# PeterCalifano/gtsam_PeterCdev

Measured on AMD Instinct MI355X. Metric: lm_iterations_per_sec, higher is better.
Workload: dtype f64; 1 GPU; bal1723; ordering=schur_nd, replicas=1, parallelism=replicas1

## Files before the change

### gtsam_petercdev_amd/csrc/handle.h

```cpp
#pragma once
#include <hip/hip_runtime.h>

#include <algorithm>
#include <new>
#include <stdexcept>
#include <string>
#include <utility>
#include <vector>

#include "gsx_internal.h"
#include "kernels.h"

#define HIPCHK(ctx, expr)                                                                  \
  do {                                                                                     \
    hipError_t e__ = (expr);                                                               \
    if (e__ != hipSuccess) {                                                               \
      (ctx)->err = std::string(#expr) + ": " + hipGetErrorString(e__);                     \
      return GSX_E_NO_DEVICE;                                                              \
    }                                                                                      \
  } while (0)

namespace gsx {

template <class Tp>
// ... 40 lines not shown
};

enum Phase { PH_LINEARIZE, PH_ASSEMBLE_H, PH_FACTORIZE, PH_BACKSOLVE, PH_LINERR, PH_RETRACT, PH_ERROR,
             PH_FACTOR_SMALL, PH_FACTOR_BIG, PH_FACTOR_LEAF, PH_K_SYRK, PH_K_TRSM, PH_K_POTRF0, PH_K_GATHER,
             PH_K_BACKSOLVE, PH_MARGINALS, PH_M_PREP, PH_M_KT, PH_M_SF, PH_M_FF, PH_M_EMIT, PH_M_LEAF, PH_COUNT };

struct Timer {
  std::vector<std::pair<hipEvent_t, hipEvent_t>> pending, pool;
  double ms = 0;
  int64_t count = 0;
};

}

namespace gsx {

struct Context {
  std::string err;
  int device = 0;
  bool has_device = false;
  hipStream_t stream = nullptr;
  HostProblem P;
  Symbolic S;
  bool has_symbolic = false;
  double relax = GSX_AMALGAMATION_AUTO;
  int relax_max_f = 128;
  std::vector<int> order;

  DevBuf<int> d_var_type, d_var_dim, d_var_state_off, d_var_tan_off, d_f_type, d_f_rows, d_f_key_ptr, d_f_vars,
      d_f_noise_kind, d_f_cols;
  DevBuf<i64> d_f_meas_off, d_f_noise_off, d_f_jac_off;
  DevBuf<double> d_meas, d_noise;
  DevBuf<FactorRec> d_frec;
  DevBuf<int> d_type_list[kNumTypeLists];
  int type_count[kNumTypeLists] = {};
  DevProblem DP{};
  int n_smart = 0;
  DevBuf<int> d_smart_slot, d_smart_status, d_smart_counters;
  DevBuf<double> d_smart_cams, d_smart_cache, d_smart_point;
  SmartDev SD{};
  void smart_begin(bool linearize) {
    if (n_smart) hipMemsetAsync(d_smart_counters.p + (linearize ? 0 : 1), 0, (linearize ? 2 : 1) * sizeof(int), stream);
  }
  DevBuf<i64> d_fr_off, d_cmap_ptr, d_gidx_ptr, d_h_off, d_hmap_ptr, d_term_ptr;
  DevBuf<TermRec> d_terms;
  DevBuf<VarRec> d_var_recs;
  DevBuf<ChildRec> d_child_recs;
  DevBuf<FrontRec> d_front_recs;
  DevBuf<i64> d_cond_last, d_cond_prev;
  DevBuf<int> d_cond_front;
  DevBuf<VarRec> d_fvar_recs;
  DevBuf<LeafRec> d_leaf_recs;
  int leaf_base = 0;
  int lin_err_slice = 0;
  DevBuf<int> d_fr_N, d_fr_F, d_fr_nfv, d_fr_fvar_ptr, d_fvars, d_fr_parent, d_fr_lean, d_fr_child_ptr, d_children, d_cmap,
      d_gidx, d_h_rows, d_hmap, d_h_loc, d_sched, d_hvars;
  DevBuf<BigDesc> d_big;
  DevSymbolic DS{};
  std::vector<std::vector<SmallLaunch>> small_launch;
  std::vector<std::vector<SmallLaunch>> leaf_launch;
  std::vector<int> leaf_max_F;
  std::vector<std::vector<SmallLaunch>> rest_launch;
  DevBuf<int> d_usched, d_rest_ids, d_tree_start, d_tree_up, d_tree_npend, d_tree_pending, d_tree_cursor;
  DevBuf<int> d_bst_roots, d_bst_child_ptr, d_bst_children, d_bst_counters;
  DevBuf<unsigned long long> d_bst_ready;
  int bst_roots = 0, bst_total = 0;
  unsigned bst_epoch = 0;
  struct TreeTier {
    int start0, nstart, max_n, threads;
    size_t med_lds;
  };
  std::vector<TreeTier> tree_tiers;
  DevBuf<i64> d_gt_dst;
  DevBuf<GatherSeg> d_gsegs;
  DevBuf<GatherSrc> d_gsrcs;
  DevBuf<int> d_gt_ld, d_gt_dims, d_gm_task, d_gm_slot, d_gm_nslots;
  DevBuf<double> d_gscratch;
  GatherArgs GA{};
  std::vector<BigLevel> big_level;
  struct ConLevel {
    int first = 0, count = 0, max_n = 0;
  };
  std::vector<ConLevel> con_level;
  std::vector<int> con_desc_of_front;
  DevBuf<ConDesc> d_con_descs;
  DevBuf<int> d_con_own_col_ptr, d_con_own_cols, d_con_own_m, d_con_child, d_con_fwd_map, d_con_iwork;
  DevBuf<i64> d_con_own_jac;
  DevBuf<double> d_con_work;
  ConTables CT{};
  int con_hd_n = 0;
  DevBuf<int> d_con_hd_tan, d_con_hd_ptr;
  DevBuf<i64> d_con_hd_jidx;
  DevBuf<double> d_con_hd_w;
  bool constrained() const { return !S.con_fronts.empty(); }
  std::vector<BigDesc> big_descs;
  int big_max_n = 0, big_max_nfv = 0;
  struct HGroup {
    int begin, count, threads, lds;
    bool global;
  };
  std::vector<HGroup> hgroups;
  DevBuf<int2> d_star_bundles;
  int n_star_bundles = 0;
  bool fused_star_env = true;
  bool fused_star = false;
  struct LeafSplit {
// ... 251 lines not shown
```

### gtsam_petercdev_amd/csrc/kernels.h

```cpp
#pragma once
#include <hip/hip_runtime.h>

#include <cstdint>
#include <vector>

#include "../../include/gsx.h"

namespace gsx {

typedef long long i64;

struct FactorRec {
  i64 jac_off;
  int s0, s1;
  int meas_off, noise_off;
  int type_kind;
  int rows_dim;
};
struct DevProblem {
  int n_vars, n_factors;
  const int *var_type, *var_dim, *var_state_off, *var_tan_off;
  const int *f_type, *f_rows, *f_key_ptr, *f_vars, *f_noise_kind, *f_cols;
  const i64 *f_meas_off, *f_noise_off, *f_jac_off;
  const double *meas, *noise;
  const FactorRec* frec;
  const int* f_active;
  int n_active;
};

struct TermRec {
  i64 jac;
  int m, colA, colB, dB, dst, pad;
};

struct VarRec {
  i64 h_off, hmap_off;
  int dA, rows, loc, toff;
};
struct LeafRec {
  i64 off, h_off, hmap_off, gidx_ptr;
  int n, F, nfv, lean;
  int dA, rows, loc, toff;
  int fvar_ptr, front, pad0, pad1;
};
constexpr int kStarMaxD = 3;
struct StarLeafRec {
  i64 off, h_off, t0;
  i64 jac0, prow_off;
  int n, nf, d, toff;
  int colA, colB, colR, dB;
  int front, jstride, rrow, pad0;
};
struct ChildRec {
  i64 src0, cmap_off;
  int nc, s1, pad0, pad1;
};
struct FrontRec {
  i64 off;
  int n, F, nfv, fvar_ptr, child_ptr, nchild;
};

struct DevSymbolic {
  int n_fronts;
  const i64* fr_off;
  const int *fr_N, *fr_F, *fr_nfv, *fr_fvar_ptr, *fvars, *fr_parent, *fr_child_ptr, *children;
  const int* fr_lean;
  const i64 *cmap_ptr, *gidx_ptr;
  const int *cmap, *gidx;
  const i64 *h_off, *hmap_ptr;
  const int *h_rows, *hmap, *h_loc;
  const i64* term_ptr;
  const TermRec* terms;
  const VarRec* var_recs;
  const ChildRec* child_recs;
  const FrontRec* front_recs;
  const VarRec* fvar_recs;
  unsigned char* wf_dirty;
  const unsigned char *wf_replaced, *wf_changed;
};
#ifdef __HIPCC__
__device__ __forceinline__ bool wildfire_skip(const DevSymbolic& S, int f, bool writer) {
  if (S.wf_dirty == nullptr) return false;
  const int p = S.fr_parent[f];
  bool dirty = (p < 0) || S.wf_dirty[p];
  if (dirty && !S.wf_replaced[f]) {
    dirty = false;
    for (int q = S.fr_fvar_ptr[f] + S.fr_nfv[f]; q < S.fr_fvar_ptr[f + 1]; ++q)
      if (S.wf_changed[S.fvars[q]]) {
        dirty = true;
        break;
      }
  }
  if (writer) S.wf_dirty[f] = dirty ? 1 : 0;
  return !dirty;
}
#endif

// ... 124 lines not shown
void launch_front_leaf(const DevProblem& P, const DevSymbolic& S, const LeafRec* recs, int count, int max_panel, int threads,
                       const double* H, const double* damp, const double* scalars, double* arena, DevStatus* status,
                       hipStream_t st);
void launch_front_star_leaf(const DevSymbolic& S, const StarLeafRec* recs, int count, const int* prow, const double* jac,
                            const double* damp, const double* scalars, double* H, double* arena, DevStatus* status,
                            hipStream_t st);
struct GatherSrc {
  i64 off;
  int d2;
  int ldF;
};
struct GatherSeg {
  i64 dst;
  i64 src;
  int n, ld, dims;
  int slot;
};
struct GatherArgs {
  const GatherSeg* segs;
  const GatherSrc* srcs;
  const i64* gt_dst;
  const int *gt_ld, *gt_dims, *gm_task, *gm_slot, *gm_nslots;
  double* scratch;
};
void launch_big_gather(const GatherArgs& G, int seg0, int nseg, int m0, int nm, double* arena, hipStream_t st);
void launch_backsolve(const DevSymbolic& S, const int* ids, int count, int threads, int max_n, const double* arena,
                      double* delta, DevStatus* status, hipStream_t st);
size_t backsolve_big_lds(int max_n, int max_F, int max_sep_rows);
void launch_backsolve_big(const DevSymbolic& S, const int* ids, int count, int max_n, int max_F, const double* arena,
                          double* delta, DevStatus* status, hipStream_t st);
bool backsolve_small_fits(int max_n, int max_F);
void launch_backsolve_small(const DevSymbolic& S, const int* ids, int count, int max_F, const double* arena, double* delta,
                            DevStatus* status, hipStream_t st);
struct BacksolveTreeArgs {
  const int* roots;
  int n_roots, n_tickets;
  const int *child_ptr, *children;
  unsigned long long* ready;
  int *head, *tail;
  unsigned epoch;
};
void launch_backsolve_tree(const DevSymbolic& S, const BacksolveTreeArgs& Q, const double* arena, double* delta,
                           DevStatus* status, hipStream_t st);
struct WildfireArgs {
  const unsigned char *replaced, *dirty;
  unsigned char* changed;
  const double* old_delta;
  DevStatus* status;
  double threshold;
};
void launch_mark_fronts(const int* ids, int count, unsigned char* flags, hipStream_t st);
void launch_wildfire_post(const DevSymbolic& S, const int* ids, int count, bool wave_per_clique, const WildfireArgs& W,
                          double* delta, hipStream_t st);
void launch_backsolve_leaf(const DevSymbolic& S, const LeafRec* recs, int count, int max_F, const double* arena,
                           double* delta, DevStatus* status, hipStream_t st);
void launch_gradient(const DevProblem& P, const DevSymbolic& S, const double* H, double* g, hipStream_t st);
void launch_ax_sqnorm(const DevProblem& P, const double* jac, const double* x, double* partials, int cap, double* scalars,
                      int slot, hipStream_t st);
void launch_vec_dot(const double* a, const double* b, int64_t n, double* partials, int cap, double* scalars, int slot,
                    hipStream_t st);
void launch_vec_axpby(double* out, double alpha, const double* a, double beta, const double* b, int64_t n, hipStream_t st);
void launch_marginal_path(const DevSymbolic& S, const int* path, int npath, int loc, int dA, int max_n, const double* arena,
                          double* out, double* Y, int64_t n_tan, hipStream_t st);
void launch_joint_cross(const double* Ya, const double* Yb, int64_t n_tan, int dA, int dB, double* out, hipStream_t st);
struct MargItem {
  int front, ti, tj, pad;
};
struct MargArgs {
  const i64 *slot, *work;
  double* cov;
  const double* arena;
  const i64* out_off;
  const int* var_dim;
  double* out;
};
void launch_marg_prep(const DevSymbolic& S, const MargArgs& M, const MargItem* items, int count, hipStream_t st);
void launch_marg_kt(const DevSymbolic& S, const MargArgs& M, const MargItem* items, int count, hipStream_t st);
void launch_marg_sf(const DevSymbolic& S, const MargArgs& M, const MargItem* items, int count, hipStream_t st);
void launch_marg_ff(const DevSymbolic& S, const MargArgs& M, const MargItem* items, int count, hipStream_t st);
void launch_marg_emit(const DevSymbolic& S, const MargArgs& M, const int2* vars, int count, hipStream_t st);
void launch_marg_leaf(const DevSymbolic& S, const MargArgs& M, const int* ids, int count, hipStream_t st);
void launch_set_scalar(double* scalars, int slot, double v, hipStream_t st);
struct ConDesc {
  i64 off;
  i64 work, fwd;
  i64 iwork;
  int N, F, K, n_fwd;
  int own_begin, own_end;
  int child_begin, child_end;
  int front;
  int fwd_map;
};
struct ConTables {
  const ConDesc* descs;
  const int *own_col_ptr, *own_cols, *own_m;
  const i64* own_jac;
  const int* child_list;
  const int* fwd_map;
  double* work;
  int* iwork;
};
void launch_constraint_fronts(const DevSymbolic& S, const ConTables& T, int first, int count, int max_n, const double* jac,
                              double* arena, DevStatus* status, hipStream_t st);
void launch_constraint_hdiag(int n, const int* tan, const int* ptr, const i64* jidx, const double* w, const double* jac,
                             double* hdiag, hipStream_t st);
constexpr int kTreeCursors = 8;
void launch_begin_factorization(double* scalars, double lambda, DevStatus* status, int* tree_cursors, hipStream_t st);
void launch_dense_partial(double* a, int n, int nf, DevStatus* status, hipStream_t st);
// ... 25 lines not shown
```

### gtsam_petercdev_amd/csrc/kernels.hip

```cpp
#include <hip/hip_runtime.h>

#include <climits>
#include <cstdio>
#include <cstdlib>

#include "device_geometry.h"
#include "gsx_internal.h"
#include "kernels.h"

namespace gsx {
using namespace gsxd;

#define T kTile

__device__ __forceinline__ double wave_sum(double v) {
#pragma unroll
  for (int o = 32; o > 0; o >>= 1) v += __shfl_down(v, o, 64);
  return v;
}
typedef double v4d __attribute__((ext_vector_type(4)));
__device__ __forceinline__ i64 readlane_i64(i64 v, int src_lane) {
  int lo = (int)(v & 0xFFFFFFFFll), hi = (int)(v >> 32);
  lo = __builtin_amdgcn_readlane(lo, src_lane);
  hi = __builtin_amdgcn_readlane(hi, src_lane);
// ... 3161 lines not shown
        acc0 += col0[r] * x;
        acc1 += col1[r] * x;
      }
#pragma unroll
      for (int o = 32; o > 0; o >>= 1) {
        acc0 += __shfl_down(acc0, o, 64);
        acc1 += __shfl_down(acc1, o, 64);
      }
      if (lane == 0) {
        y[c] = col0[n - 1] - acc0;
        if (two) y[c + 1] = col1[n - 1] - acc1;
      }
    }
#pragma unroll
    for (int q = 0; q < kTR; ++q) {
      const int e = tid + q * nt;
      if (e < w * w) {
        int r, c;
        divmod_small(e, w, rw, c, r);
        tile[r][c] = treg[q];
      }
    }
    if (tid < w) dv[tid] = dreg;
    __syncthreads();
    if (wave == 0) {
      double yr;
      if (has_inv) {
        yr = 0;
        if (lane < w) {
          yr = y[lane] * dv[lane];
          for (int r = lane + 1; r < w; ++r) yr += tile[lane][r] * y[r];
        }
      } else {
        yr = (lane < w) ? y[lane] : 0.0;
        for (int c = w - 1; c >= 0; --c) {
          const double xc = __shfl(yr, c, 64) / tile[c][c];
          if (lane == c) yr = xc;
          else if (lane < c) yr -= tile[c][lane] * xc;
        }
      }
      if (lane < w) xs[c0 + lane] = yr;
    }
    lds_barrier();
  }
  int bad = 0;
  for (int r = tid; r < F; r += nt) {
    const double x = xs[r];
    delta[gi[r]] = x;
    if (!isfinite(x)) bad = 1;
  }
  if (bad) atomicAdd(&status->n_nonfinite, 1);
}
template <int FM>
__global__ void __launch_bounds__(256) backsolve_leaf_kernel(DevSymbolic S, const LeafRec* recs, int count,
                                                             const double* arena, double* delta, DevStatus* status) {
  const int lane = threadIdx.x & 63;
  const int k = __builtin_amdgcn_readfirstlane(blockIdx.x * 4 + (threadIdx.x >> 6));
  if (k >= count) return;
  const LeafRec rec = recs[k];
  if (wildfire_skip(S, rec.front, lane == 0)) return;
  const int n = rec.n, F = rec.F;
  const double* A = arena + rec.off;
  const int* gi = S.gidx + rec.gidx_ptr;
  constexpr int U = 2;
  int g[U];
  double a[U][FM];
#pragma unroll
  for (int u = 0; u < U; ++u) {
    const int r = F + lane + 64 * u;
    const bool ok = r < n - 1;
    g[u] = ok ? gi[r] : -1;
#pragma unroll
    for (int c = 0; c < FM; ++c) a[u][c] = (ok && c < F) ? A[r + (i64)c * n] : 0.0;
  }
  const int gf = lane < F ? gi[lane] : -1;
  const int tr = lane % max(F, 1), tc = lane / max(F, 1);
  const double tri = (FM <= 8 && tc < F) ? A[tr + (i64)tc * n] : 0.0;
  const double dl = lane < F ? A[(n - 1) + (i64)lane * n] : 0.0;
  double yc[FM];
#pragma unroll
  for (int c = 0; c < FM; ++c) yc[c] = 0.0;
#pragma unroll
  for (int u = 0; u < U; ++u) {
    const double x = g[u] >= 0 ? delta[g[u]] : 0.0;
#pragma unroll
    for (int c = 0; c < FM; ++c) yc[c] = fma(a[u][c], x, yc[c]);
  }
  for (int r = F + lane + 64 * U; r < n - 1; r += 64) {
    const double x = delta[gi[r]];
#pragma unroll
    for (int c = 0; c < FM; ++c)
      if (c < F) yc[c] += A[r + (i64)c * n] * x;
  }
#pragma unroll
  for (int c = 0; c < FM; ++c) {
#pragma unroll
    for (int o = 32; o > 0; o >>= 1) yc[c] += __shfl_xor(yc[c], o, 64);
    yc[c] = tile_readlane(dl, c) - yc[c];
  }
  double xv[FM];
#pragma unroll
  for (int c = FM - 1; c >= 0; --c) {
    xv[c] = 0.0;
    if (c < F) {
      double acc = yc[c];
#pragma unroll
      for (int r = c + 1; r < FM; ++r)
        if (r < F) acc -= (FM <= 8 ? tile_readlane(tri, r + c * F) : A[r + (i64)c * n]) * xv[r];
      xv[c] = acc / (FM <= 8 ? tile_readlane(tri, c + c * F) : A[c + (i64)c * n]);
    }
  }
  double mine = 0.0;
#pragma unroll
  for (int c = 0; c < FM; ++c) mine = (lane == c) ? xv[c] : mine;
  if (lane < F) {
    delta[gf] = mine;
    if (!isfinite(mine)) atomicAdd(&status->n_nonfinite, 1);
  }
}

void launch_backsolve_leaf(const DevSymbolic& S, const LeafRec* recs, int count, int max_F, const double* arena,
                           double* delta, DevStatus* status, hipStream_t st) {
  if (!count) return;
  const int grid = (count + 3) / 4;
  if (max_F <= 4) backsolve_leaf_kernel<4><<<grid, 256, 0, st>>>(S, recs, count, arena, delta, status);
  else if (max_F <= 8) backsolve_leaf_kernel<8><<<grid, 256, 0, st>>>(S, recs, count, arena, delta, status);
  else backsolve_leaf_kernel<kLeafMaxF><<<grid, 256, 0, st>>>(S, recs, count, arena, delta, status);
}

template <bool WAVE>
__global__ void __launch_bounds__(256) wildfire_post_kernel(DevSymbolic S, const int* ids, int count, WildfireArgs W,
                                                            double* delta) {
  __shared__ int solved;
  if (threadIdx.x == 0) solved = 0;
  __syncthreads();
  const int lane = WAVE ? (threadIdx.x & 63) : 0, step = WAVE ? 64 : 1;
  const int k = WAVE ? blockIdx.x * 4 + (threadIdx.x >> 6) : blockIdx.x * 256 + threadIdx.x;
  if (k < count && W.dirty[ids[k]]) {
    const int f = ids[k];
    const int F = S.fr_F[f], nfv = S.fr_nfv[f];
    const int* gi = S.gidx + S.gidx_ptr[f];
    if (lane == 0) atomicAdd(&solved, nfv);
    bool keep = W.replaced[f] != 0;
    if (!keep) {
      double m = 0.0;
      for (int r = lane; r < F; r += step) {
        const int g = gi[r];
        m = fmax(m, fabs(W.old_delta[g] - delta[g]));
      }
      keep = WAVE ? (bool)__any(m >= W.threshold) : (m >= W.threshold);
    }
    if (keep) {
      for (int q = lane; q < nfv; q += step) W.changed[S.fvars[S.fr_fvar_ptr[f] + q]] = 1;
    } else {
      for (int r = lane; r < F; r += step) {
        const int g = gi[r];
        delta[g] = W.old_delta[g];
      }
    }
  }
  __syncthreads();
  if (threadIdx.x == 0 && solved) atomicAdd(&W.status->n_backsub, solved);
}
void launch_wildfire_post(const DevSymbolic& S, const int* ids, int count, bool wave_per_clique, const WildfireArgs& W,
                          double* delta, hipStream_t st) {
  if (count <= 0) return;
  if (wave_per_clique) wildfire_post_kernel<true><<<(count + 3) / 4, 256, 0, st>>>(S, ids, count, W, delta);
  else wildfire_post_kernel<false><<<(count + 255) / 256, 256, 0, st>>>(S, ids, count, W, delta);
}
__global__ void __launch_bounds__(256) mark_fronts_kernel(const int* ids, int count, unsigned char* flags) {
  const int k = blockIdx.x * blockDim.x + threadIdx.x;
  if (k < count) flags[ids[k]] = 1;
}
void launch_mark_fronts(const int* ids, int count, unsigned char* flags, hipStream_t st) {
  if (count > 0) mark_fronts_kernel<<<(count + 255) / 256, 256, 0, st>>>(ids, count, flags);
}

void launch_backsolve(const DevSymbolic& S, const int* ids, int count, int threads, int max_n, const double* arena,
                      double* delta, DevStatus* status, hipStream_t st) {
  static bool attr = false;
// ... 74 lines not shown
```

### gtsam_petercdev_amd/csrc/solver.hip

```cpp
#include <hip/hip_runtime.h>

#include <algorithm>
#include <cstdlib>
#include <chrono>
#include <climits>
#include <cmath>
#include <cstdio>
#include <cstring>
#include <limits>
#include <array>
#include <map>
#include <string>
#include <vector>

#include "handle.h"

using namespace gsx;

using namespace gsx;

namespace gsx {

void launch_lds_group(const DevProblem& P, const DevSymbolic& S, const int* ids, const SmallLaunch& g, const double* H,
                      const double* damp, const double* scalars, double* arena, DevStatus* status, hipStream_t st) {
// ... 221 lines not shown
    if (c->profiling > 0) timer_begin(c, PH_FACTOR_SMALL);
    const TreeArgs ta{c->d_tree_start.p + tt.start0, tt.nstart, c->d_tree_cursor.p + t, c->d_tree_pending.p,
                      c->d_tree_up.p, c->d_tree_npend.p};
    if (tt.med_lds)
      launch_front_tree_med(c->DP, c->DS, ta, tt.med_lds, c->d_H.p, c->d_damp.p, c->d_scalars.p, c->d_arena.p,
                            c->d_status.p, c->stream);
    else
      launch_front_tree(c->DP, c->DS, ta, tt.max_n, tt.threads, c->d_H.p, c->d_damp.p, c->d_scalars.p, c->d_arena.p,
                        c->d_status.p, c->stream);
    debug_sync(c, tt.med_lds ? "front_tree_med" : "front_tree", tt.nstart, (int)tt.med_lds);
    if (c->profiling > 0) timer_end(c, PH_FACTOR_SMALL);
  }
  for (int l = 0; l < S.n_ulevels; ++l) {
    for (const SmallLaunch& sl : c->rest_launch[l]) {
      if (c->profiling > 0) timer_begin(c, PH_FACTOR_SMALL);
      launch_lds_group(c->DP, c->DS, c->d_rest_ids.p + sl.begin, sl, c->d_H.p, c->d_damp.p, c->d_scalars.p, c->d_arena.p,
                       c->d_status.p, c->stream);
      debug_sync(c, sl.medium ? "front_medium (level)" : "front_small (level)", sl.count, sl.medium ? sl.max_panel : sl.max_n);
      if (c->profiling > 0) timer_end(c, PH_FACTOR_SMALL);
    }
    if (have_side && l == S.side_level0 + 1 && c->bulk_pending) {
      hipStreamWaitEvent(c->stream, c->bulk_done, 0);
      c->bulk_pending = false;
    }
    const BigLevel& B = c->big_level[l];
    const bool prof = c->profiling > 0;
    if (prof && B.count) timer_begin(c, PH_FACTOR_BIG);
    if (S.gseg_lvl_ptr[l + 1] > S.gseg_lvl_ptr[l]) {
      if (prof) timer_begin(c, PH_K_GATHER);
      launch_big_gather(c->GA, S.gseg_lvl_ptr[l], S.gseg_lvl_ptr[l + 1] - S.gseg_lvl_ptr[l], S.gm_lvl_ptr[l],
                        S.gm_lvl_ptr[l + 1] - S.gm_lvl_ptr[l], c->d_arena.p, c->stream);
      if (prof) timer_end(c, PH_K_GATHER);
    }
    if (l == 0 && have_side && !use_bulk && S.gseg_lvl_ptr[sg + 1] > S.gseg_lvl_ptr[sg]) {
      if (prof) timer_begin(c, PH_K_GATHER);
      launch_big_gather(c->GA, S.gseg_lvl_ptr[sg], S.gseg_lvl_ptr[sg + 1] - S.gseg_lvl_ptr[sg], S.gm_lvl_ptr[sg],
                        S.gm_lvl_ptr[sg + 1] - S.gm_lvl_ptr[sg], c->d_arena.p, c->stream);
      if (prof) timer_end(c, PH_K_GATHER);
    }
    if (B.count) {
      if (l == S.cap_ulevel0) shard_allreduce(c, c->d_arena.p + S.cap_begin, S.cap_end - S.cap_begin);
      if (c->con_level[l].count)
        launch_constraint_fronts(c->DS, c->CT, c->con_level[l].first, c->con_level[l].count, c->con_level[l].max_n,
                                 c->d_jac.p, c->d_arena.p, c->d_status.p, c->stream);
      dev_big_factor(c, c->d_big.p + B.begin, B.count, B.plan, c->stream, prof);
      if (prof) timer_end(c, PH_FACTOR_BIG);
    }
  }
  launch_cond_check((int)S.cond_last.size(), c->d_cond_last.p, c->d_cond_prev.p, c->d_cond_front.p, c->d_arena.p,
                    c->d_status.p, c->stream);
  timer_end(c, PH_FACTORIZE);
}

static void dev_backsolve_levels(gsx_context* c, const WildfireArgs* wf) {
  const Symbolic& S = c->S;
  timer_begin(c, PH_BACKSOLVE);
  c->delta_overwritten();
  for (int l = S.n_levels - 1; l >= 0; --l) {
    const int se = S.lvl_small_end[l];
    const struct {
      int count;
    } B{S.lvl_ptr[l + 1] - se};
    const int le = S.lvl_leaf_end[l], n_rest = S.lvl_ptr[l + 1] - le;
    int big_maxn = 0, big_maxF = 0, big_maxS = 0;
    for (int k = se; k < S.lvl_ptr[l + 1]; ++k) {
      big_maxn = std::max(big_maxn, S.N[S.sched[k]]);
      big_maxF = std::max(big_maxF, S.F[S.sched[k]]);
      big_maxS = std::max(big_maxS, S.N[S.sched[k]] - S.F[S.sched[k]]);
    }
    const bool big_own = B.count > 0 && backsolve_big_lds(big_maxn, big_maxF, big_maxS) > 0;
    if (big_own) {
      if (c->profiling > 0) timer_begin(c, PH_K_BACKSOLVE);
      launch_backsolve_big(c->DS, c->d_sched.p + se, S.lvl_ptr[l + 1] - se, big_maxn, big_maxF, c->d_arena.p, c->d_delta.p,
                           c->d_status.p, c->stream);
      if (c->profiling > 0) timer_end(c, PH_K_BACKSOLVE);
    }
    const int* small_ids = c->d_sched.p + le;
    const int n_small = se - le;
    int small_maxn = 0, small_maxF = 0;
    for (int k = le; k < se; ++k) {
      small_maxn = std::max(small_maxn, S.N[S.sched[k]]);
      small_maxF = std::max(small_maxF, S.F[S.sched[k]]);
    }
    const bool small_own = n_small > 0 && backsolve_small_fits(small_maxn, small_maxF);
    if (small_own) {
      if (c->profiling > 0) timer_begin(c, PH_K_BACKSOLVE);
      launch_backsolve_small(c->DS, small_ids, n_small, small_maxF, c->d_arena.p, c->d_delta.p, c->d_status.p,
                             c->stream);
      if (c->profiling > 0) timer_end(c, PH_K_BACKSOLVE);
    }
    const bool big_left = B.count > 0 && !big_own, small_left = n_small > 0 && !small_own;
    if (big_left && small_left && n_rest <= 512 && n_rest > B.count) {
      int maxn = 0;
      for (int k = le; k < S.lvl_ptr[l + 1]; ++k) maxn = std::max(maxn, S.N[S.sched[k]]);
      if (c->profiling > 0) timer_begin(c, PH_K_BACKSOLVE);
      launch_backsolve(c->DS, c->d_sched.p + le, n_rest, 1024, maxn, c->d_arena.p, c->d_delta.p, c->d_status.p, c->stream);
      if (c->profiling > 0) timer_end(c, PH_K_BACKSOLVE);
    } else {
      if (big_left) {
        int maxn = 0;
        for (int k = se; k < S.lvl_ptr[l + 1]; ++k) maxn = std::max(maxn, S.N[S.sched[k]]);
        if (c->profiling > 0) timer_begin(c, PH_K_BACKSOLVE);
        launch_backsolve(c->DS, c->d_sched.p + se, S.lvl_ptr[l + 1] - se, 1024, maxn, c->d_arena.p, c->d_delta.p,
                         c->d_status.p, c->stream);
        if (c->profiling > 0) timer_end(c, PH_K_BACKSOLVE);
      }
      if (small_left) {
        if (c->profiling > 0) timer_begin(c, PH_K_BACKSOLVE);
        launch_backsolve(c->DS, small_ids, n_small, small_maxn <= 48 ? 64 : 256, small_maxn, c->d_arena.p,
                         c->d_delta.p, c->d_status.p, c->stream);
        if (c->profiling > 0) timer_end(c, PH_K_BACKSOLVE);
      }
    }
    if (S.lvl_leaf_end[l] > S.lvl_ptr[l])
      launch_backsolve_leaf(c->DS, c->d_leaf_recs.p + (S.lvl_ptr[l] - c->leaf_base), S.lvl_leaf_end[l] - S.lvl_ptr[l],
                            c->leaf_max_F[l], c->d_arena.p, c->d_delta.p, c->d_status.p, c->stream);
    if (wf) {
      launch_wildfire_post(c->DS, c->d_sched.p + S.lvl_ptr[l], le - S.lvl_ptr[l], false, *wf, c->d_delta.p, c->stream);
      launch_wildfire_post(c->DS, c->d_sched.p + le, n_rest, true, *wf, c->d_delta.p, c->stream);
    }
  }
  timer_end(c, PH_BACKSOLVE);
}


void dev_backsolve(gsx_context* c, const WildfireArgs* wf) {
  static const bool levels_only = std::getenv("GSX_BS_TREE_OFF") != nullptr;
  if (wf != nullptr || levels_only) {
    dev_backsolve_levels(c, wf);
    return;
  }
  const Symbolic& S = c->S;
  timer_begin(c, PH_BACKSOLVE);
  c->delta_overwritten();
  for (int l = S.n_ulevels - 1; l >= 0; --l) {
    const int b0 = S.ulvl_ptr[l], se = S.ulvl_small_end[l], e = S.ulvl_ptr[l + 1];
    if (e > se) {
      int big_maxn = 0, big_maxF = 0, big_maxS = 0;
      for (int k = se; k < e; ++k) {
        big_maxn = std::max(big_maxn, S.N[S.usched[k]]);
        big_maxF = std::max(big_maxF, S.F[S.usched[k]]);
        big_maxS = std::max(big_maxS, S.N[S.usched[k]] - S.F[S.usched[k]]);
      }
      if (c->profiling > 0) timer_begin(c, PH_K_BACKSOLVE);
      if (backsolve_big_lds(big_maxn, big_maxF, big_maxS) > 0)
        launch_backsolve_big(c->DS, c->d_usched.p + se, e - se, big_maxn, big_maxF, c->d_arena.p, c->d_delta.p, c->d_status.p,
                             c->stream);
      else
        launch_backsolve(c->DS, c->d_usched.p + se, e - se, 1024, big_maxn, c->d_arena.p, c->d_delta.p, c->d_status.p,
                         c->stream);
      if (c->profiling > 0) timer_end(c, PH_K_BACKSOLVE);
    }
    if (se > b0) {
      int maxn = 0, maxF = 0;
      for (int k = b0; k < se; ++k) {
        maxn = std::max(maxn, S.N[S.usched[k]]);
        maxF = std::max(maxF, S.F[S.usched[k]]);
      }
      if (c->profiling > 0) timer_begin(c, PH_K_BACKSOLVE);
      if (backsolve_small_fits(maxn, maxF))
        launch_backsolve_small(c->DS, c->d_usched.p + b0, se - b0, maxF, c->d_arena.p, c->d_delta.p, c->d_status.p, c->stream);
      else
        launch_backsolve(c->DS, c->d_usched.p + b0, se - b0, maxn <= 48 ? 64 : 256, maxn, c->d_arena.p, c->d_delta.p,
                         c->d_status.p, c->stream);
      if (c->profiling > 0) timer_end(c, PH_K_BACKSOLVE);
    }
  }
  if (c->bst_total > 0) {
    hipMemsetAsync(c->d_bst_counters.p, 0, 2 * sizeof(int), c->stream);
    if (++c->bst_epoch == 0) c->bst_epoch = 1;
    if (c->profiling > 0) timer_begin(c, PH_K_BACKSOLVE);
    launch_backsolve_tree(c->DS,
                          BacksolveTreeArgs{c->d_bst_roots.p, c->bst_roots, c->bst_total, c->d_bst_child_ptr.p,
                                            c->d_bst_children.p, c->d_bst_ready.p, c->d_bst_counters.p,
                                            c->d_bst_counters.p + 1, c->bst_epoch},
                          c->d_arena.p, c->d_delta.p, c->d_status.p, c->stream);
    if (c->profiling > 0) timer_end(c, PH_K_BACKSOLVE);
    debug_sync(c, "backsolve_tree", c->bst_roots, c->bst_total);
  }
  if (S.n_levels > 0 && S.lvl_leaf_end[0] > S.lvl_ptr[0])
    launch_backsolve_leaf(c->DS, c->d_leaf_recs.p + (S.lvl_ptr[0] - c->leaf_base), S.lvl_leaf_end[0] - S.lvl_ptr[0],
                          c->leaf_max_F[0], c->d_arena.p, c->d_delta.p, c->d_status.p, c->stream);
  timer_end(c, PH_BACKSOLVE);
}

void dev_linear_error(gsx_context* c, bool solved_step) {
  static const bool direct_env = std::getenv("GSX_LINERR_DIRECT") != nullptr;
  const bool direct_only = direct_env || c->constrained() || c->use_pcg();
  timer_begin(c, PH_LINERR);
  if (solved_step && !direct_only && c->h_ready) {
    if (!c->lin0_ready) {
      launch_lin0(c->DP, c->d_jac.p, c->d_partials.p, gsx_context::kPartials, c->d_scalars.p, c->stream);
      c->lin0_computed();
    }
    launch_model_error(c->DP, c->DS, c->d_hvars.p, (int)c->hv_list.size(), c->d_H.p, c->d_delta.p, c->d_damp.p,
                       c->d_partials.p, gsx_context::kPartials, c->d_scalars.p, c->stream);
  } else {
    launch_linear_error(c->DP, c->d_jac.p, c->d_delta.p, c->d_partials.p, gsx_context::kPartials, c->d_scalars.p,
                        c->lin_err_slice, c->stream);
  }
  c->sc_dirty |= (1u << SC_LIN0) | (1u << SC_LIND);
  timer_end(c, PH_LINERR);
}
void dev_retract(gsx_context* c, const double* d_delta) {
  timer_begin(c, PH_RETRACT);
  launch_retract(c->DP, c->d_values.p, d_delta, c->d_trial.p, c->stream);
  timer_end(c, PH_RETRACT);
}
void dev_error(gsx_context* c, const double* d_vals, int slot) {
  timer_begin(c, PH_ERROR);
  const int* lists[kNumTypeLists];
  for (int k = 0; k < kNumTypeLists; ++k) lists[k] = c->d_type_list[k].p;
  c->smart_begin(false);
  launch_error(c->DP, lists, c->type_count, d_vals, c->d_partials.p, gsx_context::kPartials, c->d_scalars.p, slot, c->stream,
               &c->SD);
  c->sc_dirty |= 1u << slot;
  timer_end(c, PH_ERROR);
}
gsx_status readback(gsx_context* c) {
  if (c->sharded() && c->sc_dirty) {
    launch_shard_pack(c->d_scalars.p, c->d_status.p, c->sc_dirty, c->d_xscal.p, c->stream);
    shard_allreduce(c, c->d_xscal.p, kXScalars);
    launch_shard_unpack(c->d_xscal.p, c->sc_dirty, c->d_scalars.p, c->d_status.p, c->stream);
  }
  c->sc_dirty = 0;
  if (c->shard_failed) {
    c->shard_failed = false;
    c->err = "the all-reduce callback of a sharded handle failed";
    return GSX_E_NO_DEVICE;
  }
  HIPCHK(c, hipMemcpyAsync(c->h_scalars, c->d_scalars.p, SC_COUNT * sizeof(double), hipMemcpyDeviceToHost, c->stream));
  HIPCHK(c, hipMemcpyAsync(c->h_status, c->d_status.p, sizeof(DevStatus), hipMemcpyDeviceToHost, c->stream));
  HIPCHK(c, hipStreamSynchronize(c->stream));
  HIPCHK(c, hipGetLastError());
  c->n_cheirality = c->h_status->n_cheirality;
// ... 108 lines not shown
}

void direct_solve(gsx_context* c, HMode hm, int diagonal, double mind, double maxd, double lambda, bool backsolve) {
  if (hm == H_ALWAYS || (hm == H_IF_STALE && !c->h_ready)) dev_assemble_h(c);
  dev_damping(c, diagonal, mind, maxd);
  dev_factorize(c, lambda);
  if (backsolve) dev_backsolve(c);
}
gsx_status damped_step(gsx_context* c, HMode hm, int diagonal, double mind, double maxd, double lambda) {
  if (!c->use_pcg()) {
    direct_solve(c, hm, diagonal, mind, maxd, lambda, true);
    return GSX_OK;
  }
  if (diagonal && (hm == H_ALWAYS || (hm == H_IF_STALE && !c->h_ready))) dev_assemble_h(c);
  dev_damping(c, diagonal, mind, maxd);
  return pcg_solve(c, lambda, c->pcg_params, nullptr, nullptr);
}

gsx_status compute_error_sync(gsx_context* c, double* out) {
  dev_error(c, c->d_values.p, SC_ERR);
  gsx_status st = readback(c);
  if (st != GSX_OK) return st;
  *out = c->h_scalars[SC_ERR];
  return GSX_OK;
}

}

extern "C" {

const char* gsx_version(void) { return "gsx 0.1.0 (gfx950)"; }

int32_t gsx_device_count(void) {
  int n = 0;
  if (hipGetDeviceCount(&n) != hipSuccess) return 0;
  return n;
}

gsx_status gsx_create(const gsx_problem_desc* desc, int32_t device, gsx_handle* out) {
  if (!out) return GSX_E_INVALID;
  *out = nullptr;
  gsx_context* c = new gsx_context();
  gsx_status st = lower_problem(desc, c->P, c->err);
  if (st != GSX_OK) {
    std::fprintf(stderr, "gsx_create: %s\n", c->err.c_str());
    delete c;
    return st;
  }
  c->n_smart = (int)std::count(c->P.f_type.begin(), c->P.f_type.end(), (int)GSX_F_SMART_PROJECTION);
  c->device = device;
  {
    const char* e = std::getenv("GSX_FUSED_STAR");
    c->fused_star_env = !(e && std::atoi(e) == 0);
  }
  int n = 0;
  if (hipGetDeviceCount(&n) == hipSuccess && n > 0 && device >= 0 && device < n && hipSetDevice(device) == hipSuccess &&
      hipStreamCreate(&c->stream) == hipSuccess) {
    c->has_device = true;
    st = upload_problem(c);
    if (st != GSX_OK) {
      std::fprintf(stderr, "gsx_create: %s\n", c->err.c_str());
      delete c;
      return st;
    }
  }
  *out = c;
  return GSX_OK;
}

gsx_status gsx_destroy(gsx_handle h) {
  if (!h) return GSX_OK;
  if (h->has_device) {
    hipSetDevice(h->device);
    hipStreamSynchronize(h->stream);
    for (auto& t : h->timers) {
      for (auto& ev : t.pending) t.pool.push_back(ev);
      for (auto& ev : t.pool) {
        hipEventDestroy(ev.first);
        hipEventDestroy(ev.second);
      }
    }
    if (h->bulk) {
      hipStreamSynchronize(h->bulk);
      hipStreamDestroy(h->bulk);
      if (h->bulk_go) hipEventDestroy(h->bulk_go);
      if (h->bulk_done) hipEventDestroy(h->bulk_done);
    }
    if (h->h_scalars) hipHostFree(h->h_scalars);
    if (h->h_status) hipHostFree(h->h_status);
    pcg_work_destroy(h->pcg);
    h->pcg = nullptr;
  }
  hipStream_t st = h->stream;
  const bool dev = h->has_device;
  delete h;
  if (dev && st) hipStreamDestroy(st);
  return GSX_OK;
}

const char* gsx_last_error(gsx_handle h) { return h ? h->err.c_str() : ""; }

gsx_status gsx_set_ordering(gsx_handle h, const uint64_t* keys, int32_t n) {
  if (!h || (!keys && n > 0)) return GSX_E_INVALID;
  if (n != h->P.n_vars) {
    h->err = "ordering size differs from the number of variables";
    return GSX_E_BAD_ORDERING;
// ... 951 lines not shown
```

### gtsam_petercdev_amd/csrc/upload.hip

```cpp
#include <hip/hip_runtime.h>

#include <algorithm>
#include <cstdlib>
#include <chrono>
#include <climits>
#include <cmath>
#include <cstdio>
#include <cstring>
#include <limits>
#include <array>
#include <map>
#include <string>
#include <vector>

#include "handle.h"

using namespace gsx;

namespace gsx {

int factor_type_list(const HostProblem& P, int f) {
  const int kp = P.f_key_ptr[f], nk = P.f_key_ptr[f + 1] - kp;
  return type_list_of(P.f_type[f], nk > 0 ? P.types[P.f_vars[kp]] : -1, nk > 1 ? P.types[P.f_vars[kp + 1]] : -1,
                      P.f_meas_ptr[f + 1] - P.f_meas_ptr[f]);
// ... 244 lines not shown
  HIPCHK(c, c->d_gidx_ptr.upload(std::vector<i64>(S.gidx_ptr.begin(), S.gidx_ptr.end()), st));
  HIPCHK(c, c->d_cmap.upload(S.cmap, st));
  HIPCHK(c, c->d_gidx.upload(S.gidx, st));
  HIPCHK(c, c->d_h_off.upload(std::vector<i64>(S.h_off.begin(), S.h_off.end()), st));
  HIPCHK(c, c->d_hmap_ptr.upload(std::vector<i64>(S.hmap_ptr.begin(), S.hmap_ptr.end()), st));
  HIPCHK(c, c->d_h_rows.upload(S.h_rows, st));
  HIPCHK(c, c->d_hmap.upload(S.hmap, st));
  HIPCHK(c, c->d_h_loc.upload(S.h_loc, st));
  HIPCHK(c, c->d_term_ptr.upload(std::vector<i64>(S.term_ptr.begin(), S.term_ptr.end()), st));
  {
    std::vector<TermRec> terms(S.t_jac.size());
    for (size_t i = 0; i < terms.size(); ++i)
      terms[i] = TermRec{(i64)S.t_jac[i], S.t_m[i], S.t_colA[i], S.t_colB[i], S.t_dB[i], S.t_dst[i], 0};
    HIPCHK(c, c->d_terms.upload(terms, st));
    std::vector<VarRec> vrec(P.n_vars);
    for (int v = 0; v < P.n_vars; ++v)
      vrec[v] = VarRec{(i64)S.h_off[v], (i64)S.hmap_ptr[v], P.dims[v], S.h_rows[v], S.h_loc[v], P.tan_off[v]};
    std::vector<ChildRec> crec(S.children.size());
    for (size_t i = 0; i < crec.size(); ++i) {
      const int ch = S.children[i];
      crec[i] = ChildRec{(i64)S.off[ch] + (i64)S.F[ch] * S.N[ch] + S.F[ch], (i64)S.cmap_ptr[ch], S.N[ch],
                         S.N[ch] - S.F[ch], 0, 0};
    }
    std::vector<VarRec> fvrec(S.fvars.size());
    for (size_t i = 0; i < fvrec.size(); ++i) fvrec[i] = vrec[S.fvars[i]];
    std::vector<FrontRec> frec(S.n_fronts);
    for (int f = 0; f < S.n_fronts; ++f)
      frec[f] = FrontRec{(i64)S.off[f], S.N[f], S.F[f], S.nfrontal_vars[f], S.fvar_ptr[f], S.child_ptr[f],
                         S.child_ptr[f + 1] - S.child_ptr[f]};
    HIPCHK(c, c->d_var_recs.upload(vrec, st));
    HIPCHK(c, c->d_child_recs.upload(crec, st));
    HIPCHK(c, c->d_front_recs.upload(frec, st));
    HIPCHK(c, c->d_cond_last.upload(std::vector<i64>(S.cond_last.begin(), S.cond_last.end()), st));
    HIPCHK(c, c->d_cond_prev.upload(std::vector<i64>(S.cond_prev.begin(), S.cond_prev.end()), st));
    HIPCHK(c, c->d_cond_front.upload(S.cond_front, st));
    HIPCHK(c, c->d_fvar_recs.upload(fvrec, st));
    HIPCHK(c, hipStreamSynchronize(st));
  }
  HIPCHK(c, c->d_sched.upload(S.sched, st));
  {
    const int b = S.n_levels ? S.lvl_ptr[0] : 0, e = S.n_levels ? S.lvl_leaf_end[0] : 0;
    std::vector<LeafRec> lr((size_t)std::max(e - b, 0));
    for (int k = b; k < e; ++k) {
      const int f = S.sched[k];
      const int v0 = S.fvars[S.fvar_ptr[f]];
      lr[k - b] = LeafRec{(i64)S.off[f], (i64)S.h_off[v0], (i64)S.hmap_ptr[v0], (i64)S.gidx_ptr[f],
                          S.N[f], S.F[f], S.nfrontal_vars[f], (int)S.lean[f],
                          P.dims[v0], S.h_rows[v0], S.h_loc[v0], P.tan_off[v0],
                          S.fvar_ptr[f], f, 0, 0};
    }
    c->leaf_base = b;
    c->h_leaf_recs = lr;
    HIPCHK(c, c->d_leaf_recs.upload(lr, st));
  }
  HIPCHK(c, c->d_H.alloc(std::max<int64_t>(S.h_size, 1)));
  HIPCHK(c, c->d_arena.alloc(std::max<int64_t>(S.arena_size, 1)));
  {
    struct VI {
      int v, psize;
      int64_t terms;
    };
    std::vector<VI> light, heavy, huge, diag, star, tile;
    static const bool tile_off = std::getenv("GSX_H_TILE_OFF") != nullptr;
    auto is_tile = [&](int v) {
      const int64_t tb = S.term_ptr[v], te = S.term_ptr[v + 1];
      if (tile_off || te - tb < 2 || te - tb > 64 || (int64_t)S.h_rows[v] * P.dims[v] * 8 * 4 > 48 * 1024) return false;
      int64_t t = tb;
      while (t < te) {
        int64_t e = t + 1;
        while (e < te && S.t_jac[e] == S.t_jac[t]) ++e;
        if (S.t_m[t] > 8 || S.t_dB[e - 1] != 1 || S.t_dst[e - 1] != S.h_rows[v] - 1 || S.t_colB[e - 1] + 1 > 16) return false;
        t = e;
      }
      return true;
    };
    std::vector<int> star_dst;
    auto is_star = [&](int v) {
      const int64_t tb = S.term_ptr[v], te = S.term_ptr[v + 1];
      if (te - tb < 3 || (te - tb) % 3 != 0 || P.dims[v] > 7) return false;
      star_dst.clear();
      for (int64_t t = tb; t < te; t += 3) {
        star_dst.push_back(S.t_dst[t + 1]);
        if (S.t_dst[t] != 0 || S.t_dst[t + 2] != S.h_rows[v] - 1 || S.t_dB[t + 2] != 1) return false;
        if (S.t_dst[t + 1] == 0 || S.t_dst[t + 1] == S.h_rows[v] - 1) return false;
        if (S.t_m[t] != S.t_m[tb] || S.t_colA[t] != S.t_colA[tb] || S.t_colB[t + 1] != S.t_colB[tb + 1] ||
            S.t_dB[t + 1] != S.t_dB[tb + 1] || S.t_colB[t + 2] != S.t_colB[tb + 2] || S.t_jac[t] != S.t_jac[t + 1] ||
            S.t_jac[t] != S.t_jac[t + 2])
          return false;
      }
      std::sort(star_dst.begin(), star_dst.end());
      return std::adjacent_find(star_dst.begin(), star_dst.end()) == star_dst.end();
    };
    for (int v = 0; v < P.n_vars; ++v) {
      if (!S.scheduled[S.front_of_var[v]]) continue;
      const int psize = S.h_rows[v] * P.dims[v];
      const int64_t terms = S.term_ptr[v + 1] - S.term_ptr[v];
      if (is_star(v)) {
        star.push_back({v, psize, terms});
        continue;
      }
      if (terms >= 64 && S.h_rows[v] == P.dims[v] + 1 && P.dims[v] <= 15) diag.push_back({v, psize, terms});
      else if (is_tile(v)) tile.push_back({v, psize, terms});
      else if (terms >= 96 && (int64_t)psize * 4 * 8 <= 48 * 1024) heavy.push_back({v, psize, terms});
      else if ((int64_t)psize * 8 <= 48 * 1024) light.push_back({v, psize, terms});
      else huge.push_back({v, psize, terms});
    }
// ... 450 lines not shown
```

Baseline: 589.1 LM iterations/s.

## Pack multiple small leaf backsolves per wavefront using 16/32-lane groups

Level-0 leaf cliques are sorted by size class at upload, and a new packed device routine solves 4 or 2 small leaves per 64-lane wave using lane subgroups with xor-shuffle reductions. Larger leaves keep the previous one-wave-per-leaf path, and the kernel dispatches by block index across the three classes. This aims to cut idle lanes and launch width in the leaf backsolve, at the cost of an extra sorted record buffer and more complex kernel code, with an environment switch to disable it.

```diff
diff --git a/gtsam_petercdev_amd/csrc/handle.h b/gtsam_petercdev_amd/csrc/handle.h
--- a/gtsam_petercdev_amd/csrc/handle.h
+++ b/gtsam_petercdev_amd/csrc/handle.h
@@ -116,6 +116,9 @@
   DevBuf<VarRec> d_fvar_recs;
   DevBuf<LeafRec> d_leaf_recs;
   int leaf_base = 0;
+  bool bs_leaf_pack_env = true;
+  DevBuf<LeafRec> d_leaf_bs_recs;
+  int leaf_bs_n[3] = {0, 0, 0};
   int lin_err_slice = 0;
   DevBuf<int> d_fr_N, d_fr_F, d_fr_nfv, d_fr_fvar_ptr, d_fvars, d_fr_parent, d_fr_lean, d_fr_child_ptr, d_children, d_cmap,
       d_gidx, d_h_rows, d_hmap, d_h_loc, d_sched, d_hvars;
diff --git a/gtsam_petercdev_amd/csrc/kernels.h b/gtsam_petercdev_amd/csrc/kernels.h
--- a/gtsam_petercdev_amd/csrc/kernels.h
+++ b/gtsam_petercdev_amd/csrc/kernels.h
@@ -43,6 +43,11 @@
   int dA, rows, loc, toff;
   int fvar_ptr, front, pad0, pad1;
 };
+struct LeafPack {
+  int n16, n32, n64, nb16, nb32;
+};
+constexpr int kLeafPackRows = 4;
+static_assert(16 * kLeafPackRows <= 64 && 32 * kLeafPackRows <= 128, "classes of backsolve_leaf_packed");
 constexpr int kStarMaxD = 3;
 struct StarLeafRec {
   i64 off, h_off, t0;
@@ -273,8 +278,9 @@
 void launch_mark_fronts(const int* ids, int count, unsigned char* flags, hipStream_t st);
 void launch_wildfire_post(const DevSymbolic& S, const int* ids, int count, bool wave_per_clique, const WildfireArgs& W,
                           double* delta, hipStream_t st);
-void launch_backsolve_leaf(const DevSymbolic& S, const LeafRec* recs, int count, int max_F, const double* arena,
-                           double* delta, DevStatus* status, hipStream_t st);
+int leaf_pack_class(int n, int F, int max_F);
+void launch_backsolve_leaf(const DevSymbolic& S, const LeafRec* recs, int n16, int n32, int n64, int max_F,
+                           const double* arena, double* delta, DevStatus* status, hipStream_t st);
 void launch_gradient(const DevProblem& P, const DevSymbolic& S, const double* H, double* g, hipStream_t st);
 void launch_ax_sqnorm(const DevProblem& P, const double* jac, const double* x, double* partials, int cap, double* scalars,
                       int slot, hipStream_t st);
diff --git a/gtsam_petercdev_amd/csrc/kernels.hip b/gtsam_petercdev_amd/csrc/kernels.hip
--- a/gtsam_petercdev_amd/csrc/kernels.hip
+++ b/gtsam_petercdev_amd/csrc/kernels.hip
@@ -3237,10 +3237,9 @@
   if (bad) atomicAdd(&status->n_nonfinite, 1);
 }
 template <int FM>
-__global__ void __launch_bounds__(256) backsolve_leaf_kernel(DevSymbolic S, const LeafRec* recs, int count,
-                                                             const double* arena, double* delta, DevStatus* status) {
+__device__ __forceinline__ void backsolve_leaf_wave(const DevSymbolic& S, const LeafRec* recs, int count, int k,
+                                                    const double* arena, double* delta, DevStatus* status) {
   const int lane = threadIdx.x & 63;
-  const int k = __builtin_amdgcn_readfirstlane(blockIdx.x * 4 + (threadIdx.x >> 6));
   if (k >= count) return;
   const LeafRec rec = recs[k];
   if (wildfire_skip(S, rec.front, lane == 0)) return;
@@ -3303,14 +3302,116 @@
     if (!isfinite(mine)) atomicAdd(&status->n_nonfinite, 1);
   }
 }
-
-void launch_backsolve_leaf(const DevSymbolic& S, const LeafRec* recs, int count, int max_F, const double* arena,
-                           double* delta, DevStatus* status, hipStream_t st) {
-  if (!count) return;
-  const int grid = (count + 3) / 4;
-  if (max_F <= 4) backsolve_leaf_kernel<4><<<grid, 256, 0, st>>>(S, recs, count, arena, delta, status);
-  else if (max_F <= 8) backsolve_leaf_kernel<8><<<grid, 256, 0, st>>>(S, recs, count, arena, delta, status);
-  else backsolve_leaf_kernel<kLeafMaxF><<<grid, 256, 0, st>>>(S, recs, count, arena, delta, status);
+template <int FM, int G>
+__device__ __forceinline__ void backsolve_leaf_packed(const DevSymbolic& S, const LeafRec* recs, int count, int k0,
+                                                      const double* arena, double* delta, DevStatus* status) {
+  static_assert(FM <= 8 && (G == 16 || G == 32), "the triangle travels in F * F <= G lanes");
+  const int lane = threadIdx.x & 63, lp = lane & (G - 1), base = lane - lp;
+  const int k = k0 + lane / G;
+  if (k >= count) return;
+  const LeafRec* rec = recs + k;
+  if (wildfire_skip(S, rec->front, lp == 0)) return;
+  const int n = rec->n, F = rec->F;
+  const double* A = arena + rec->off;
+  const int* gi = S.gidx + rec->gidx_ptr;
+  constexpr int R = kLeafPackRows, NA = 64 / G;
+  int g[R];
+  double a[R][FM];
+#pragma unroll
+  for (int j = 0; j < R; ++j) {
+    const int r = F + lp + G * j;
+    const bool ok = r < n - 1;
+    g[j] = ok ? gi[r] : -1;
+#pragma unroll
+    for (int c = 0; c < FM; ++c) a[j][c] = (ok && c < F) ? A[r + (i64)c * n] : 0.0;
+  }
+  const int gf = lp < F ? gi[lp] : -1;
+  const int tr = lp % max(F, 1), tc = lp / max(F, 1);
+  const double tri = tc < F ? A[tr + (i64)tc * n] : 0.0;
+  const double dl = lp < F ? A[(n - 1) + (i64)lp * n] : 0.0;
+  double x[R];
+#pragma unroll
+  for (int j = 0; j < R; ++j) x[j] = g[j] >= 0 ? delta[g[j]] : 0.0;
+  double yc[FM];
+#pragma unroll
+  for (int c = 0; c < FM; ++c) {
+    double acc[NA];
+#pragma unroll
+    for (int i = 0; i < NA; ++i) acc[i] = 0.0;
+#pragma unroll
+    for (int j = 0; j < R; ++j) acc[j % NA] = fma(a[j][c], x[j], acc[j % NA]);
+    if (R <= NA) {
+#pragma unroll
+      for (int i = 0; i < NA; ++i) acc[i] += 0.0;
+    }
+#pragma unroll
+    for (int h = NA / 2; h > 0; h >>= 1)
+#pragma unroll
+      for (int i = 0; i < h; ++i) acc[i] += acc[i + h];
+    yc[c] = acc[0];
+#pragma unroll
+    for (int o = G / 2; o > 0; o >>= 1) yc[c] += __shfl_xor(yc[c], o, 64);
+    yc[c] = __shfl(dl, base + c, 64) - yc[c];
+  }
+  double xv[FM];
+#pragma unroll
+  for (int c = FM - 1; c >= 0; --c) {
+    xv[c] = 0.0;
+    const double tcc = __shfl(tri, base + min(c + c * F, G - 1), 64);
+    double acc = yc[c];
+#pragma unroll
+    for (int r = c + 1; r < FM; ++r) {
+      const double trc = __shfl(tri, base + min(r + c * F, G - 1), 64);
+      if (r < F) acc -= trc * xv[r];
+    }
+    if (c < F) xv[c] = acc / tcc;
+  }
+  double mine = 0.0;
+#pragma unroll
+  for (int c = 0; c < FM; ++c) mine = (lp == c) ? xv[c] : mine;
+  if (lp < F) {
+    delta[gf] = mine;
+    if (!isfinite(mine)) atomicAdd(&status->n_nonfinite, 1);
+  }
+}
+
+template <int FM>
+__global__ void __launch_bounds__(256) backsolve_leaf_kernel(DevSymbolic S, const LeafRec* recs, LeafPack pk,
+                                                             const double* arena, double* delta, DevStatus* status) {
+  const int wave = __builtin_amdgcn_readfirstlane(threadIdx.x >> 6);
+  int b = blockIdx.x;
+  if constexpr (FM <= 8) {
+    if (b < pk.nb16) {
+      backsolve_leaf_packed<FM, 16>(S, recs, pk.n16, (b * 4 + wave) * 4, arena, delta, status);
+      return;
+    }
+    b -= pk.nb16;
+    if (b < pk.nb32) {
+      backsolve_leaf_packed<FM, 32>(S, recs + pk.n16, pk.n32, (b * 4 + wave) * 2, arena, delta, status);
+      return;
+    }
+    b -= pk.nb32;
+    recs += pk.n16 + pk.n32;
+  }
+  backsolve_leaf_wave<FM>(S, recs, pk.n64, b * 4 + wave, arena, delta, status);
+}
+
+int leaf_pack_class(int n, int F, int max_F) {
+  const int sep = n - 1 - F;
+  if (max_F > 8) return 64;
+  if (sep <= 16 * kLeafPackRows && F * F <= 16) return 16;
+  if (sep <= 32 * kLeafPackRows && F * F <= 32) return 32;
+  return 64;
+}
+
+void launch_backsolve_leaf(const DevSymbolic& S, const LeafRec* recs, int n16, int n32, int n64, int max_F,
+                           const double* arena, double* delta, DevStatus* status, hipStream_t st) {
+  if (n16 + n32 + n64 == 0) return;
+  const LeafPack pk{n16, n32, n64, (n16 + 15) / 16, (n32 + 7) / 8};
+  const int grid = pk.nb16 + pk.nb32 + (n64 + 3) / 4;
+  if (max_F <= 4) backsolve_leaf_kernel<4><<<grid, 256, 0, st>>>(S, recs, pk, arena, delta, status);
+  else if (max_F <= 8) backsolve_leaf_kernel<8><<<grid, 256, 0, st>>>(S, recs, pk, arena, delta, status);
+  else backsolve_leaf_kernel<kLeafMaxF><<<grid, 256, 0, st>>>(S, recs, pk, arena, delta, status);
 }
 
 template <bool WAVE>
diff --git a/gtsam_petercdev_amd/csrc/solver.hip b/gtsam_petercdev_amd/csrc/solver.hip
--- a/gtsam_petercdev_amd/csrc/solver.hip
+++ b/gtsam_petercdev_amd/csrc/solver.hip
@@ -297,6 +297,17 @@
   timer_end(c, PH_FACTORIZE);
 }
 
+static void backsolve_leaves(gsx_context* c, int l) {
+  const Symbolic& S = c->S;
+  const int n = S.lvl_leaf_end[l] - S.lvl_ptr[l];
+  if (l == 0 && c->leaf_bs_n[0] + c->leaf_bs_n[1] > 0)
+    launch_backsolve_leaf(c->DS, c->d_leaf_bs_recs.p, c->leaf_bs_n[0], c->leaf_bs_n[1], c->leaf_bs_n[2], c->leaf_max_F[0],
+                          c->d_arena.p, c->d_delta.p, c->d_status.p, c->stream);
+  else
+    launch_backsolve_leaf(c->DS, c->d_leaf_recs.p + (S.lvl_ptr[l] - c->leaf_base), 0, 0, n, c->leaf_max_F[l], c->d_arena.p,
+                          c->d_delta.p, c->d_status.p, c->stream);
+}
+
 static void dev_backsolve_levels(gsx_context* c, const WildfireArgs* wf) {
   const Symbolic& S = c->S;
   timer_begin(c, PH_BACKSOLVE);
@@ -358,8 +369,7 @@
       }
     }
     if (S.lvl_leaf_end[l] > S.lvl_ptr[l])
-      launch_backsolve_leaf(c->DS, c->d_leaf_recs.p + (S.lvl_ptr[l] - c->leaf_base), S.lvl_leaf_end[l] - S.lvl_ptr[l],
-                            c->leaf_max_F[l], c->d_arena.p, c->d_delta.p, c->d_status.p, c->stream);
+      backsolve_leaves(c, l);
     if (wf) {
       launch_wildfire_post(c->DS, c->d_sched.p + S.lvl_ptr[l], le - S.lvl_ptr[l], false, *wf, c->d_delta.p, c->stream);
       launch_wildfire_post(c->DS, c->d_sched.p + le, n_rest, true, *wf, c->d_delta.p, c->stream);
@@ -424,8 +434,7 @@
     debug_sync(c, "backsolve_tree", c->bst_roots, c->bst_total);
   }
   if (S.n_levels > 0 && S.lvl_leaf_end[0] > S.lvl_ptr[0])
-    launch_backsolve_leaf(c->DS, c->d_leaf_recs.p + (S.lvl_ptr[0] - c->leaf_base), S.lvl_leaf_end[0] - S.lvl_ptr[0],
-                          c->leaf_max_F[0], c->d_arena.p, c->d_delta.p, c->d_status.p, c->stream);
+    backsolve_leaves(c, 0);
   timer_end(c, PH_BACKSOLVE);
 }
 
@@ -640,6 +649,8 @@
   {
     const char* e = std::getenv("GSX_FUSED_STAR");
     c->fused_star_env = !(e && std::atoi(e) == 0);
+    e = std::getenv("GSX_BS_LEAF_PACK");
+    c->bs_leaf_pack_env = !(e && std::atoi(e) == 0);
   }
   int n = 0;
   if (hipGetDeviceCount(&n) == hipSuccess && n > 0 && device >= 0 && device < n && hipSetDevice(device) == hipSuccess &&
diff --git a/gtsam_petercdev_amd/csrc/upload.hip b/gtsam_petercdev_amd/csrc/upload.hip
--- a/gtsam_petercdev_amd/csrc/upload.hip
+++ b/gtsam_petercdev_amd/csrc/upload.hip
@@ -320,6 +320,19 @@
     c->leaf_base = b;
     c->h_leaf_recs = lr;
     HIPCHK(c, c->d_leaf_recs.upload(lr, st));
+    int max_F = 0, cnt[3] = {0, 0, 0};
+    auto cls = [&](const LeafRec& r) { const int g = leaf_pack_class(r.n, r.F, max_F); return g == 16 ? 0 : g == 32 ? 1 : 2; };
+    for (const LeafRec& r : lr) max_F = std::max(max_F, r.F);
+    if (c->bs_leaf_pack_env)
+      for (const LeafRec& r : lr) ++cnt[cls(r)];
+    c->leaf_bs_n[0] = c->leaf_bs_n[1] = c->leaf_bs_n[2] = 0;
+    if (cnt[0] + cnt[1] > 0) {
+      std::vector<LeafRec> br(lr.size());
+      size_t at[3] = {0, (size_t)cnt[0], (size_t)cnt[0] + cnt[1]};
+      for (const LeafRec& r : lr) br[at[cls(r)]++] = r;
+      for (int q = 0; q < 3; ++q) c->leaf_bs_n[q] = cnt[q];
+      HIPCHK(c, c->d_leaf_bs_recs.upload(br, st));
+    }
   }
   HIPCHK(c, c->d_H.alloc(std::max<int64_t>(S.h_size, 1)));
   HIPCHK(c, c->d_arena.alloc(std::max<int64_t>(S.arena_size, 1)));
```

After: 601.5 LM iterations/s, median of 6. +2.1%, better.
